# zenoran/sesameai-tts

Hardware: AMD Instinct MI355X
Metric: audio frames/sec (higher is better)
Workload: dtype bf16

## Files before the change

sesameai-tts_amd/csrc/dec_persist.cuh:

```cuda
#pragma once
#include "gemv.cuh"
#include "sampler.cuh"

#define DP_NB 256
#ifndef DP_NREP
#define DP_NREP 8
#endif
#define DP_TIMEOUT 5000000ull
#define DP_NL 4
#define DP_D 1024
#define DP_FFN 8192
#define DP_HD 128
#define DP_NQKV 1536
#define DP_WSM_ROWS 2560
#define DP_W2S_U4 (256L * 4 * 1024)
#define DP_W13P_U4 (256L * 4 * 32 * 64)
#define DP_LSLOTS 1088

typedef __attribute__((address_space(3))) uint32_t dp_lu32;
typedef __attribute__((address_space(3))) volatile uint32_t dp_lvu32;
typedef __attribute__((address_space(3))) u32x4_t dp_lu4;
typedef __attribute__((address_space(3))) unsigned short dp_lu16;
typedef __attribute__((address_space(3))) float dp_lf32;
typedef __attribute__((address_space(4))) const uint32_t dp_cu32;
// ... 14 lines not shown
    const bf16_t* proj_emb;
    const bf16_t* qkv0_tab;
    const bf16_t *hdec, *qd;
    const bf16_t *kc, *vc;
    long kv_layer_stride;
    float temperature; int topk;
    const bf16_t* noise;
    const uint64_t* rng;
    const SlotSampling* slot_tab;
    int slot_row0;
    const int* forced;
    int V, ncb;
    int* frame;
    bf16_t* logits_out;
    int cb_first, cb_last;
    dp_u64 *gQ, *gH1, *gH2, *gL, *gP;
    uint32_t* err;
    uint32_t* epoch;
    float eps;
    int trickle_sleep, poll_sleep;
    int fault;
    dp_u64* stamps;
};

#ifdef DP_TIMELINE
#define DP_STAMPS(a_) ((a_).stamps)
#define DP_FAULT(a_) ((a_).fault)
#else
#define DP_STAMPS(a_) ((dp_u64*)nullptr)
#define DP_FAULT(a_) 0
#endif
#define DP_OFF_K 0
#define DP_OFF_V 65536
#define DP_OFF_U 131072
#define DP_OFF_XA (DP_OFF_U)
#define DP_OFF_XC (DP_OFF_U + 2048)
#define DP_OFF_QB (DP_OFF_U + 4096)
#define DP_OFF_ATT (DP_OFF_U + 6144)
#define DP_CAND_SLOTS 2112
#define DP_OFF_CANDT (DP_OFF_U)
#define DP_OFF_CANDI (DP_OFF_U + DP_CAND_SLOTS * 4)
#define DP_OFF_LOGITS (DP_OFF_U + 16896)
#define DP_OFF_SMAX (DP_OFF_LOGITS + 5120)
#define DP_OFF_PS (DP_OFF_SMAX + 1024)
#define DP_OFF_MISC (DP_OFF_PS + 1024)
#define DP_LDS_BYTES (DP_OFF_MISC + 512)
static_assert(DP_OFF_CANDI + DP_CAND_SLOTS * 4 <= DP_OFF_LOGITS, "sampler candidate lists overrun the LDS logits");
#define DP_M_HL 0
#define DP_M_H0 16
#define DP_M_H1 18
#define DP_M_FXA 20
#define DP_M_FQ 21
#define DP_M_FXC 22
#define DP_M_FLG 23
#define DP_M_FTOK 24
#define DP_M_ATTN 25
#define DP_M_CD 26
#define DP_M_BAR 27
#define DP_M_ABORT 28
#define DP_M_TOK 29
#define DP_M_SBV 32
#define DP_M_SBI 36
#define DP_M_SN 40
#define DP_M_STOK 41
#define DP_M_SWTOT 42
#define DP_M_RNG 112
#define DP_M_SARG 116
#define DP_M_TILE 48

enum { DP_E_Q = 0, DP_E_H1 = 1, DP_E_P = 2, DP_E_H2 = 3, DP_E_L = 4 };
__device__ __forceinline__ uint32_t dp_tag(uint32_t base, int s, int l, int e) { return base + 1u + (uint32_t)((s * DP_NL + l) * 5 + e); }

__device__ __forceinline__ void dp_gran_store(dp_u64* p, uint32_t tag, uint32_t val) {
    __hip_atomic_store(p, ((dp_u64)tag << 32) | val, __ATOMIC_RELAXED, __HIP_MEMORY_SCOPE_AGENT);
}
__device__ __forceinline__ dp_u64 dp_gran_load(const dp_u64* p) { return __hip_atomic_load(p, __ATOMIC_RELAXED, __HIP_MEMORY_SCOPE_AGENT); }

__device__ __forceinline__ bool dp_give_up(dp_u64 t0, dp_lvu32* ab, uint32_t* err, uint32_t code, int lane) {
    if (*ab) return true;
    if (__builtin_amdgcn_s_memrealtime() - t0 > DP_TIMEOUT) {
        *ab = 1;
        if (lane == 0) atomicCAS(err, 0u, code);
        return true;
    }
    return false;
}

template <int N, bool AT_LEAST, class Issue>
__device__ __forceinline__ bool dp_wait(dp_lvu32* f, uint32_t tag, dp_lvu32* ab, uint32_t* err, uint32_t code, int lane, int sleep_units, Issue issue) {
    auto hit = [&]() { const uint32_t v = *f; return AT_LEAST ? (int32_t)(v - tag) >= 0 : v == tag; };
    int seen = (int)hit();
#pragma unroll
    for (int k = 0; k < N; ++k) {
        issue(k);
        const int nap = seen ? 0 : sleep_units;
        for (int z = 0; z < nap; ++z) __builtin_amdgcn_s_sleep(1);
        seen |= (int)hit();
    }
    seen = __builtin_amdgcn_readfirstlane(seen);
    if (!seen) {
        const dp_u64 t0 = __builtin_amdgcn_s_memrealtime();
        for (uint32_t spins = 1; !hit(); ++spins)
            if ((spins & 255u) == 0 && dp_give_up(t0, ab, err, code, lane)) return false;
    }
    asm volatile("" ::: "memory");
    return true;
}

template <int NL>
__device__ __forceinline__ bool dp_sweep(const dp_u64* g, int n_valid, uint32_t tag, uint32_t (&v)[2 * NL], int lane, dp_lvu32* ab, uint32_t* err,
                                         uint32_t code, int poll_sleep, dp_u64* passes = nullptr) {
    const dp_u64 t0 = __builtin_amdgcn_s_memrealtime();
    const int last_pair = (n_valid - 1) >> 1;
    for (;;) {
        if (passes && lane == 0) *passes += 1;
        u32x4_t x[NL];
#pragma unroll
        for (int j = 0; j < NL; ++j) {
            const dp_u64* p = g + 2 * min(j * 64 + lane, last_pair);
            asm volatile("global_load_dwordx4 %0, %1, off sc1" : "=v"(x[j]) : "v"(p) : "memory");
// ... 100 lines not shown
    mx0 = wave_max(mx0);
    float l0 = 0.f;
#pragma unroll
    for (int i = 0; i < NG; ++i) {
        s0[i] = (s0[i] == -INFINITY) ? 0.f : __expf(s0[i] - mx0);
        l0 += s0[i];
        if (sub == 0) myps[4 * i + grp] = s0[i];
    }
    l0 = wave_sum(l0) * (1.0f / 16.0f);
    asm volatile("s_waitcnt lgkmcnt(0)" ::: "memory");
    float o00 = 0.f, o01 = 0.f;
#pragma unroll
    for (int t4 = 0; t4 < NG; ++t4) {
        const u32x4_t p4 = *reinterpret_cast<const __attribute__((address_space(3))) u32x4_t*>(myps + 4 * t4);
        const float pw[4] = {__uint_as_float(p4.x), __uint_as_float(p4.y), __uint_as_float(p4.z), __uint_as_float(p4.w)};
        uint32_t vr[4];
#pragma unroll
        for (int u = 0; u < 4; ++u) vr[u] = vt[(4 * t4 + u) * 64 + lane];
#pragma unroll
        for (int u = 0; u < 4; ++u) { o00 += pw[u] * lo2f(vr[u]); o01 += pw[u] * hi2f(vr[u]); }
    }
    const float i0 = 1.0f / l0;
    att[h * 64 + lane] = pack_bf(o00 * i0, o01 * i0);
}
__device__ __forceinline__ void dp_attention_wave(char* lds, int wave, int l, int cb, int lane) {
    dp_lu32* misc = (dp_lu32*)(lds + DP_OFF_MISC);
    const int kvh = wave >> 2;
    const dp_lu4* qb = (const dp_lu4*)(lds + DP_OFF_QB);
    const dp_lu4* kt = (const dp_lu4*)(lds + DP_OFF_K + ((l * 2 + kvh) * 32) * 256);
    const dp_lu32* vt = (const dp_lu32*)(lds + DP_OFF_V + ((l * 2 + kvh) * 32) * 256);
    dp_lf32* ps = (dp_lf32*)(lds + DP_OFF_PS) + wave * 32;
    dp_lu32* att = (dp_lu32*)(lds + DP_OFF_ATT);
    dp_attention_head(qb, kt, vt, ps, att, wave, cb + 1, 0.08838834764831845f, lane);
    asm volatile("s_waitcnt lgkmcnt(0)" ::: "memory");
    if (lane == 0) __hip_atomic_fetch_add(misc + DP_M_ATTN, 1u, __ATOMIC_RELAXED, __HIP_MEMORY_SCOPE_WORKGROUP);
}

struct DpQuadSync {
    dp_lvu32* ctr; dp_lvu32* ab; uint32_t* err; int lane; uint32_t* phase; dp_u64* stamp;
    __device__ __forceinline__ void mark(int i) const { if (stamp != nullptr && lane == 0) stamp[i] = __builtin_amdgcn_s_memrealtime(); }
    __device__ __forceinline__ void operator()() const {
        asm volatile("s_waitcnt lgkmcnt(0)" ::: "memory");
        const uint32_t want = 4u * (++*phase);
        if (lane == 0) __hip_atomic_fetch_add((dp_lu32*)ctr, 1u, __ATOMIC_RELAXED, __HIP_MEMORY_SCOPE_WORKGROUP);
        const dp_u64 t0 = __builtin_amdgcn_s_memrealtime();
        for (uint32_t spins = 1; (int32_t)(*ctr - want) < 0; ++spins) {
            __builtin_amdgcn_s_sleep(2);
            if ((spins & 255u) == 0 && dp_give_up(t0, ab, err, 0xB00u, lane)) break;
        }
        asm volatile("" ::: "memory");
    }
};

template <bool DEBUG_OUT>
__device__ __forceinline__ int dp_sample_step(const DecPersistArgs& a, char* lds, int qw, int lane, int cu, int cb, int s, uint32_t* quad_phase) {
    dp_lu32* misc = (dp_lu32*)(lds + DP_OFF_MISC);
    dp_lvu32* ab = (dp_lvu32*)(misc + DP_M_ABORT);
    const int tid = qw * 64 + lane;
    if (DP_STAMPS(a) != nullptr && cu == 100 && tid == 0) DP_STAMPS(a)[s * 32 + 22] = __builtin_amdgcn_s_memrealtime();
    const dp_lu4* lg = (const dp_lu4*)(lds + DP_OFF_LOGITS);
    uint32_t w[2][4];
    {
        const uint4 v0 = dp_ldq(lg + tid);
        w[0][0] = v0.x; w[0][1] = v0.y; w[0][2] = v0.z; w[0][3] = v0.w;
        const uint4 v1 = tid < 64 ? dp_ldq(lg + 256 + tid) : make_uint4(0, 0, 0, 0);
        w[1][0] = v1.x; w[1][1] = v1.y; w[1][2] = v1.z; w[1][3] = v1.w;
    }
    if (DEBUG_OUT && a.logits_out != nullptr && cu == 0) {
        for (int i = lane; i < a.V; i += 64) a.logits_out[(long)cb * a.V + i] = ((const dp_lu16*)lg)[i];
    }
    SampleScratch sc;
    sc.cand_t = (lds_f32_t*)(lds + DP_OFF_CANDT); sc.cand_i = (lds_i32_t*)(lds + DP_OFF_CANDI); sc.s_max = (lds_u32_t*)(lds + DP_OFF_SMAX); sc.cand_q = (lds_f32_t*)(lds + DP_OFF_SMAX);
    sc.s_bv = (lds_f32_t*)(misc + DP_M_SBV); sc.s_bi = (lds_i32_t*)(misc + DP_M_SBI); sc.s_n = (lds_i32_t*)(misc + DP_M_SN);
    sc.s_tok = (lds_i32_t*)(misc + DP_M_STOK); sc.s_wtot = (lds_i32_t*)(misc + DP_M_SWTOT);
    DpQuadSync sync{(dp_lvu32*)(misc + DP_M_BAR), ab, a.err, lane, quad_phase, DP_STAMPS(a) != nullptr && cu == 100 && qw == 0 ? DP_STAMPS(a) + 4352 + s * 16 : nullptr};
    const uint64_t seed = (uint64_t)misc[DP_M_RNG] | ((uint64_t)misc[DP_M_RNG + 1] << 32), step = (uint64_t)misc[DP_M_RNG + 2] | ((uint64_t)misc[DP_M_RNG + 3] << 32);
    const int sV = (int)misc[DP_M_SARG], sK = (int)misc[DP_M_SARG + 2];
    const float sT = __uint_as_float(misc[DP_M_SARG + 1]);
    const bool sN = misc[DP_M_SARG + 3] != 0u;
    int tok = 0;
#ifdef DP_TIMELINE
    const int reps = (a.trickle_sleep & 128) ? 2 : 1;
#else
    constexpr int reps = 1;
#endif
#pragma unroll 1
    for (int r = 0; r < reps; ++r) {
        sync.mark(6);
        tok = sample_body<2>(w, sV, sT, sK, sN ? a.noise + (long)cb * sV : nullptr, seed, step, 0, cb, sc, tid, sync);
        sync.mark(7);
    }
    if (DP_STAMPS(a) != nullptr && cu == 100 && tid == 0) DP_STAMPS(a)[s * 32 + 23] = __builtin_amdgcn_s_memrealtime();
    if (tid == 0 && cu == 0) a.frame[cb] = tok;
    return tok;
}

typedef __attribute__((ext_vector_type(8))) __bf16 dp_bf16x8;
typedef __attribute__((ext_vector_type(4))) float dp_f32x4;
template <bool HAS_TILE, int NBK, int TROLE>
__device__ __forceinline__ void dp_compute_wave(const DecPersistArgs& a, char* lds, const int wave, const unsigned lane, const int cu, const uint32_t base,
                                                const uint32_t ropev) {
    constexpr bool HAS_B = !HAS_TILE;
    const bool is_x = HAS_TILE && TROLE == 1, is_a = HAS_TILE ? TROLE == 2 : TROLE == 1, is_b = HAS_B && !is_a;
    constexpr int NT = HAS_TILE ? 32 : 0, NCD = NT + NBK * 4, N1 = NCD / 3;
    dp_lu32* misc = (dp_lu32*)(lds + DP_OFF_MISC);
    dp_lvu32* ab = (dp_lvu32*)(misc + DP_M_ABORT);
    const int ts = a.trickle_sleep & 63;
    const int unit = is_a ? cu * 3 + (wave - 2) : cu * 2 + (wave - 5);
    auto my_block = [&](int b) { return wave < 4 ? wave + 4 * b : min((wave + 4) + 3 * b, wave == 6 ? 13 : 15); };
    const int hunit = is_x ? -1 : (wave < 6 ? cu * 4 + (wave - 2) : (cu < 2 ? 1024 + cu : -1));
    const int hrow0 = hunit < 0 ? 0 : 2 * hunit, hrow1 = hunit < 0 ? 0 : min(2 * hunit + 1, a.V - 1);
    uint4 wsa[2][2], wsb[HAS_B ? 2 : 1][2];
    uint4 wt[HAS_TILE ? 32 : 1];
    uint4 wd[NBK][4];

    auto ws_row = [&](int slot, int cb, int k) -> const bf16_t* {
        if (slot < DP_NL && !is_x) {
            if (is_a) {
                const int row = 2 * unit + (k >> 1);
                return a.wsm + ((long)slot * DP_WSM_ROWS + row) * DP_D;
            }
            return a.wsm + ((long)slot * DP_WSM_ROWS + DP_NQKV + 2 * unit + (k >> 1)) * DP_D;
        }
        return a.head_t + ((long)(cb - 1) * a.V + ((k >> 1) ? hrow1 : hrow0)) * DP_D;
    };
    auto load_wsa = [&](int slot, int cb, int k) { wsa[k >> 1][k & 1] = reinterpret_cast<const uint4*>(ws_row(slot, cb, k))[(k & 1) * 64 + lane]; };
    auto load_wsb = [&](int slot, int cb, int k) { wsb[HAS_B ? k >> 1 : 0][k & 1] = reinterpret_cast<const uint4*>(ws_row(slot, cb, k))[(k & 1) * 64 + lane]; };
// ... 97 lines not shown
                        tile[(lane >> 4) * 4 + 0] = acc[0]; tile[(lane >> 4) * 4 + 1] = acc[1];
                        tile[(lane >> 4) * 4 + 2] = acc[2]; tile[(lane >> 4) * 4 + 3] = acc[3];
                    }
                    asm volatile("s_waitcnt lgkmcnt(0)" ::: "memory");
                    if (lane < 8) {
                        const uint32_t hv = dp_swiglu(tile[lane], tile[8 + lane]);
                        ((dp_lu16*)(misc + DP_M_HL))[wave * 8 + lane] = (unsigned short)hv;
                    }
                }
                asm volatile("s_waitcnt lgkmcnt(0)" ::: "memory");
                if (lane == 0) __hip_atomic_fetch_add(misc + DP_M_CD, 1u, __ATOMIC_RELAXED, __HIP_MEMORY_SCOPE_WORKGROUP);
                {
                    const uint32_t want = 7u * (uint32_t)(it + 1);
                    const dp_u64 t0 = __builtin_amdgcn_s_memrealtime();
                    for (uint32_t spins = 1; (int32_t)(*(dp_lvu32*)(misc + DP_M_CD) - want) < 0; ++spins)
                        if ((spins & 255u) == 0 && dp_give_up(t0, ab, a.err, 0x950u, lane)) return;
                    asm volatile("" ::: "memory");
                }
                if (st0) DP_STAMPS(a)[4096 + s * 8 + 4] = __builtin_amdgcn_s_memrealtime();
                uint4 h[4];
#pragma unroll
                for (int q = 0; q < 4; ++q) h[q] = dp_ldq((const dp_lu4*)(misc + DP_M_HL) + q);
#pragma unroll
                for (int b = 0; b < NBK; ++b) {
                    const int n = my_block(b) * 64 + lane;
                    const float p = dp_down_partial(wd[b], h);
                    dp_gran_store(a.gP + ((long)(n >> 2) * 256 + cu) * 4 + (n & 3), dp_tag(base, s, l, DP_E_P), __float_as_uint(p));
                }
                if (st0) DP_STAMPS(a)[4096 + s * 8 + 5] = __builtin_amdgcn_s_memrealtime();
            }
        }
        {
            if (!dp_wait<1, false>((dp_lvu32*)(misc + DP_M_FXA), dp_tag(base, s, DP_NL - 1, DP_E_H2), ab, a.err, 0x960u, lane, ts, [&](int) {})) return;
            const bool st2 = DP_STAMPS(a) != nullptr && cu == 100 && lane == 0 && wave == 2;
            if (st2) DP_STAMPS(a)[s * 32 + 20] = __builtin_amdgcn_s_memrealtime();
            if (hunit >= 0) {
                const dp_lu4* xs = (const dp_lu4*)(lds + DP_OFF_XA);
                const uint4 x0 = dp_ldq(xs + lane), x1 = dp_ldq(xs + 64 + lane);
                uint4 r00 = wsa[0][0], r01 = wsa[0][1], r10 = wsa[1][0], r11 = wsa[1][1];
                if (HAS_B && is_b) { r00 = wsb[0][0]; r01 = wsb[0][1]; r10 = wsb[HAS_B ? 1 : 0][0]; r11 = wsb[HAS_B ? 1 : 0][1]; }
                float a0 = dot8(r00, x0, 0.f); a0 = dot8(r01, x1, a0);
                float a1 = dot8(r10, x0, 0.f); a1 = dot8(r11, x1, a1);
                a0 = wave_sum(a0); a1 = wave_sum(a1);
                if (lane < DP_NREP) dp_gran_store(a.gL + lane * DP_LSLOTS + hunit, dp_tag(base, s, DP_NL - 1, DP_E_L), pack_bf(a0, a1));
            }
            if (st2) DP_STAMPS(a)[s * 32 + 21] = __builtin_amdgcn_s_memrealtime();
            if (DP_STAMPS(a) != nullptr && s == 5 && lane == 0 && hunit >= 0) DP_STAMPS(a)[1024 + cu * 8 + wave] = __builtin_amdgcn_s_memrealtime();
            if (HAS_B) {
#pragma unroll
                for (int k = 0; k < 4; ++k) load_wsb(0, cb, k);
            }
        }
        if (!HAS_TILE) {
            if (!dp_wait<1, false>((dp_lvu32*)(misc + DP_M_FLG), dp_tag(base, s, DP_NL - 1, DP_E_L), ab, a.err, 0x970u, lane, ts, [&](int) {})) return;
            (void)dp_sample_step<false>(a, lds, wave - 4, (int)lane, cu, cb, s, &quad_phase);
            if (*ab) return;
        }
    }
}

#ifndef CSM_DEC_PERSIST_ELSEWHERE
static __global__ __launch_bounds__(512) void k_dec_persist(const DecPersistArgs a) {
    extern __shared__ __attribute__((aligned(16))) char lds[];
    const int wave = __builtin_amdgcn_readfirstlane(threadIdx.x >> 6), cu = blockIdx.x;
    const unsigned lane = threadIdx.x & 63;
    dp_lu32* misc = (dp_lu32*)(lds + DP_OFF_MISC);
    dp_lvu32* ab = (dp_lvu32*)(misc + DP_M_ABORT);
    uint32_t ropev = 0;
    if (wave >= 2 && wave <= 4 && lane < 32) {
        const int row = 2 * (cu * 3 + (wave - 2));
        const int e = (row < 1024 ? row : row - 1024) % DP_HD;
        ropev = reinterpret_cast<const uint32_t*>(a.rope)[lane * (DP_HD / 2) + e / 2];
    }
    for (int i = threadIdx.x; i < 128; i += 512) misc[i] = 0;
    for (int i = threadIdx.x; i < 2560 / 2; i += 512) ((dp_lu32*)(lds + DP_OFF_LOGITS))[i] = 0;
    for (int i = threadIdx.x; i < 131072 / 16; i += 512) dp_stq((dp_lu4*)lds + i, make_uint4(0, 0, 0, 0));
    __syncthreads();
    {
        const int npos = a.cb_first + 1;
        for (int i = threadIdx.x; i < DP_NL * 2 * npos * 16; i += 512) {
            const int c = i & 15, pos = (i >> 4) % npos, lk = (i >> 4) / npos;
            const long src = (long)(lk >> 1) * a.kv_layer_stride + ((long)(lk & 1) * 32 + pos) * DP_HD;
            dp_stq((dp_lu4*)(lds + DP_OFF_K + (lk * 32 + pos) * 256) + c, reinterpret_cast<const uint4*>(a.kc + src)[c]);
            dp_stq((dp_lu4*)(lds + DP_OFF_V + (lk * 32 + pos) * 256) + c, reinterpret_cast<const uint4*>(a.vc + src)[c]);
        }
        for (int i = threadIdx.x; i < 128; i += 512) dp_stq((dp_lu4*)(lds + DP_OFF_QB) + i, reinterpret_cast<const uint4*>(a.qd)[i]);
        if (threadIdx.x < 2) misc[DP_M_H0 + threadIdx.x] = reinterpret_cast<const uint32_t*>(a.hdec)[2 * cu + threadIdx.x];
        const uint32_t* se = a.slot_tab != nullptr ? reinterpret_cast<const uint32_t*>(a.slot_tab + a.slot_row0) : nullptr;
        const bool has = se != nullptr && se[1] != 0u, own = has && se[2] != 0u;
        if (threadIdx.x >= 64 && threadIdx.x < 68) misc[DP_M_RNG + threadIdx.x - 64] = own ? se[4 + threadIdx.x - 64] : (a.rng ? reinterpret_cast<const uint32_t*>(a.rng)[threadIdx.x - 64] : 0u);
        if (threadIdx.x == 128) { misc[DP_M_SARG] = (uint32_t)a.V; misc[DP_M_SARG + 1] = has ? se[0] : __float_as_uint(a.temperature); misc[DP_M_SARG + 2] = has ? se[1] : (uint32_t)a.topk; misc[DP_M_SARG + 3] = a.noise != nullptr; }
    }
    __syncthreads();
    const uint32_t base = dp_sload32(a.epoch);
    if (wave == 7) {
        __builtin_amdgcn_s_setprio(2);
        const int rep = cu % DP_NREP, ln = (int)lane;
        const dp_u64 *rgQ = a.gQ + rep * 768, *rgH1 = a.gH1 + rep * 512, *rgH2 = a.gH2 + rep * 512, *rgL = a.gL + rep * DP_LSLOTS;
        const dp_u64* rgP = a.gP + (long)cu * 1024;
        const int n_steps = a.cb_last - a.cb_first + 1;
        uint32_t quad_phase = 0;
        dp_flag((dp_lvu32*)(misc + DP_M_FQ), dp_tag(base, 0, 0, DP_E_Q));
        const bool st = DP_STAMPS(a) != nullptr && cu == 100 && lane == 0;
#define DP_STAMP(s_, i_) do { if (st) DP_STAMPS(a)[(s_) * 32 + (i_)] = __builtin_amdgcn_s_memrealtime(); } while (0)
        for (int s = 0; s < n_steps; ++s) {
            const int cb = a.cb_first + s;
            for (int l = 0; l < DP_NL; ++l) {
                if (l > 0) {
                    {
                        uint32_t v[8];
                        const uint4 g0 = reinterpret_cast<const uint4*>(a.norms + (long)(2 * l) * DP_D)[ln], g1 = reinterpret_cast<const uint4*>(a.norms + (long)(2 * l) * DP_D)[64 + ln];
                        if (!dp_sweep<4>(rgH2, 512, dp_tag(base, s, l - 1, DP_E_H2), v, ln, ab, a.err, 0x100u + l, a.poll_sleep)) return;
#pragma unroll
                        for (int j = 0; j < 4; ++j) { ((dp_lu32*)(lds + DP_OFF_XA))[2 * (j * 64 + ln)] = v[2 * j]; ((dp_lu32*)(lds + DP_OFF_XA))[2 * (j * 64 + ln) + 1] = v[2 * j + 1]; }
                        dp_norm_in_lds((dp_lu4*)(lds + DP_OFF_XA), g0, g1, a.eps, ln);
                        dp_flag((dp_lvu32*)(misc + DP_M_FXA), dp_tag(base, s, l - 1, DP_E_H2));
                        DP_STAMP(s, l * 4 + 0);
                    }
                    {
                        uint32_t v[12];
                        if (!dp_sweep<6>(rgQ, 768, dp_tag(base, s, l, DP_E_Q), v, ln, ab, a.err, 0x200u + l, a.poll_sleep, st ? DP_STAMPS(a) + s * 32 + 26 : nullptr)) return;
#pragma unroll
                        for (int j = 0; j < 4; ++j) { ((dp_lu32*)(lds + DP_OFF_QB))[2 * (j * 64 + ln)] = v[2 * j]; ((dp_lu32*)(lds + DP_OFF_QB))[2 * (j * 64 + ln) + 1] = v[2 * j + 1]; }
                        {
                            const int kvh = ln >> 5, wd_ = 2 * (ln & 31);
                            dp_lu32* kr = (dp_lu32*)(lds + DP_OFF_K + ((l * 2 + kvh) * 32 + cb) * 256);
                            dp_lu32* vr = (dp_lu32*)(lds + DP_OFF_V + ((l * 2 + kvh) * 32 + cb) * 256);
                            kr[wd_] = v[8]; kr[wd_ + 1] = v[9]; vr[wd_] = v[10]; vr[wd_ + 1] = v[11];
                        }
                        dp_flag((dp_lvu32*)(misc + DP_M_FQ), dp_tag(base, s, l, DP_E_Q));
                        DP_STAMP(s, l * 4 + 1);
                    }
                }
                dp_attention_wave(lds, 7, l, cb, ln);
                {
                    uint32_t v[8];
                    const uint4 g0 = reinterpret_cast<const uint4*>(a.norms + (long)(2 * l + 1) * DP_D)[ln], g1 = reinterpret_cast<const uint4*>(a.norms + (long)(2 * l + 1) * DP_D)[64 + ln];
                    if (!dp_sweep<4>(rgH1, 512, dp_tag(base, s, l, DP_E_H1), v, ln, ab, a.err, 0x300u + l, a.poll_sleep)) return;
#pragma unroll
                    for (int j = 0; j < 4; ++j) { ((dp_lu32*)(lds + DP_OFF_XC))[2 * (j * 64 + ln)] = v[2 * j]; ((dp_lu32*)(lds + DP_OFF_XC))[2 * (j * 64 + ln) + 1] = v[2 * j + 1]; }
                    dp_norm_in_lds((dp_lu4*)(lds + DP_OFF_XC), g0, g1, a.eps, ln);
                    dp_flag((dp_lvu32*)(misc + DP_M_FXC), dp_tag(base, s, l, DP_E_H1));
                    DP_STAMP(s, l * 4 + 2);
                }
                {
                    uint32_t v[16];
                    if (!dp_sweep<8>(rgP, 1024, dp_tag(base, s, l, DP_E_P), v, ln, ab, a.err, 0x400u + l, a.poll_sleep, st ? DP_STAMPS(a) + s * 32 + 27 : nullptr)) return;
                    float t0_, t1_;
                    dp_reduce_partials(v, t0_, t1_);
                    const uint32_t h1w = *(dp_lvu32*)(misc + DP_M_H1 + (ln & 1));
                    float y0, y1;
                    {
#pragma clang fp contract(off)
                        y0 = round_bf(t0_) + lo2f(h1w); y1 = round_bf(t1_) + hi2f(h1w);
                    }
                    const uint32_t pair = pack_bf(y0, y1);
                    if (ln < 2) misc[DP_M_H0 + ln] = pair;
                    if (ln < 2 * DP_NREP) dp_gran_store(a.gH2 + (ln >> 1) * 512 + 2 * cu + (ln & 1), dp_tag(base, s, l, DP_E_H2), pair);
                    DP_STAMP(s, l * 4 + 3);
                }
            }
            {
                uint32_t v[8];
                const uint4 g0 = reinterpret_cast<const uint4*>(a.dec_norm)[ln], g1 = reinterpret_cast<const uint4*>(a.dec_norm)[64 + ln];
                if (!dp_sweep<4>(rgH2, 512, dp_tag(base, s, DP_NL - 1, DP_E_H2), v, ln, ab, a.err, 0x500u, a.poll_sleep, st ? DP_STAMPS(a) + s * 32 + 25 : nullptr)) return;
#pragma unroll
                for (int j = 0; j < 4; ++j) { ((dp_lu32*)(lds + DP_OFF_XA))[2 * (j * 64 + ln)] = v[2 * j]; ((dp_lu32*)(lds + DP_OFF_XA))[2 * (j * 64 + ln) + 1] = v[2 * j + 1]; }
                dp_norm_in_lds((dp_lu4*)(lds + DP_OFF_XA), g0, g1, a.eps, ln);
                dp_flag((dp_lvu32*)(misc + DP_M_FXA), dp_tag(base, s, DP_NL - 1, DP_E_H2));
                DP_STAMP(s, 16);
                if (DP_STAMPS(a) != nullptr && s == 5 && lane == 0) DP_STAMPS(a)[1024 + 2048 + 256 + cu] = __builtin_amdgcn_s_memrealtime();
            }
            {
                uint32_t v[18];
                const int ng = (a.V + 1) / 2;
                if (!dp_sweep<9>(rgL, ng, dp_tag(base, s, DP_NL - 1, DP_E_L), v, ln, ab, a.err, 0x600u, a.poll_sleep, st ? DP_STAMPS(a) + s * 32 + 24 : nullptr)) return;
#pragma unroll
                for (int j = 0; j < 9; ++j) {
                    const int g0 = 2 * (j * 64 + ln);
                    if (g0 < ng) ((dp_lu32*)(lds + DP_OFF_LOGITS))[g0] = v[2 * j];
                    if (g0 + 1 < ng) ((dp_lu32*)(lds + DP_OFF_LOGITS))[g0 + 1] = v[2 * j + 1];
                }
                if ((a.V & 1) && ln == 0) ((dp_lu16*)(lds + DP_OFF_LOGITS))[a.V] = 0;
                dp_flag((dp_lvu32*)(misc + DP_M_FLG), dp_tag(base, s, DP_NL - 1, DP_E_L));
                DP_STAMP(s, 17);
                if (DP_STAMPS(a) != nullptr && s == 5 && lane == 0) DP_STAMPS(a)[1024 + 2048 + cu] = __builtin_amdgcn_s_memrealtime();
            }
            {
                const int tok = dp_sample_step<true>(a, lds, 3, ln, cu, cb, s, &quad_phase);
                if (*ab) return;
                DP_STAMP(s, 18);
                if (cb + 1 < a.ncb) {
                    int fed = a.forced ? a.forced[cb] : tok;
                    fed = min(max(fed, 0), a.V - 1);
                    const uint32_t* hrow = reinterpret_cast<const uint32_t*>(a.proj_emb + ((long)cb * a.V + fed) * DP_D);
                    const uint32_t* qrow = reinterpret_cast<const uint32_t*>(a.qkv0_tab + ((long)(cb - 1) * a.V + fed) * DP_NQKV);
                    uint32_t qv[12];
#pragma unroll
                    for (int j = 0; j < 12; ++j) qv[j] = qrow[j * 64 + ln];
                    const uint32_t hv = ln < 2 ? hrow[2 * cu + ln] : 0u;
#pragma unroll
                    for (int j = 0; j < 8; ++j) ((dp_lu32*)(lds + DP_OFF_QB))[j * 64 + ln] = qv[j];
#pragma unroll
                    for (int j = 8; j < 12; ++j)
                        ((dp_lu32*)(lds + (j < 10 ? DP_OFF_K : DP_OFF_V) + ((j & 1) * 32 + cb + 1) * 256))[ln] = qv[j];
                    if (ln < 2) misc[DP_M_H0 + ln] = hv;
                    dp_flag((dp_lvu32*)(misc + DP_M_FQ), dp_tag(base, s + 1, 0, DP_E_Q));
                    DP_STAMP(s, 19);
                }
            }
        }
        if (cu == 0 && lane == 0) __hip_atomic_store(a.epoch, base + (uint32_t)(n_steps * DP_NL * 5 + 8), __ATOMIC_RELAXED, __HIP_MEMORY_SCOPE_AGENT);
        return;
    }
    if (wave < 2) dp_compute_wave<true, 2, 1>(a, lds, wave, lane, cu, base, ropev);
    else if (wave < 4) dp_compute_wave<true, 2, 2>(a, lds, wave, lane, cu, base, ropev);
    else if (wave == 4) dp_compute_wave<false, 3, 1>(a, lds, wave, lane, cu, base, ropev);
    else dp_compute_wave<false, 3, 2>(a, lds, wave, lane, cu, base, ropev);
}
#endif

static __global__ void k_dp_pack_gateup(const bf16_t* w1, const bf16_t* w3, uint4* out) {
    const long i = (long)blockIdx.x * blockDim.x + threadIdx.x;
    if (i >= 256L * 4 * 32 * 64) return;
    const int lane = (int)(i & 63), t = (int)((i >> 6) & 31), q = (int)((i >> 11) & 3), c = (int)(i >> 13);
    const int r = lane & 15, pair = c * 32 + 8 * q + (r & 7);
    const bf16_t* w = r < 8 ? w1 : w3;
    out[i] = *reinterpret_cast<const uint4*>(w + (long)pair * DP_D + 32 * t + 8 * (lane >> 4));
}

static __global__ void k_dp_retile_w2(const bf16_t* w2, uint4* w2s) {
    const long i = (long)blockIdx.x * blockDim.x + threadIdx.x;
    if (i >= 256L * 4 * 1024) return;
    const int n = (int)(i % 1024), q = (int)((i / 1024) % 4), c = (int)(i / 4096);
    w2s[i] = *reinterpret_cast<const uint4*>(w2 + (long)n * DP_FFN + c * 32 + q * 8);
}

hipError_t csm_launch_dec_persist(const DecPersistArgs& p, hipStream_t st);
const void* csm_dec_persist_kernel();
```

sesameai-tts_amd/csrc/sampler.cuh:

```cuda
#pragma once
#include "common.cuh"
#include <math.h>

static __global__ __launch_bounds__(256) void k_embed_sum(const int* tokens , const uint8_t* mask ,
                                                   const bf16_t* text_emb, const bf16_t* audio_emb,
                                                   int audio_vocab, int text_vocab, int ncb, int d,
                                                   bf16_t* h ) {
    __shared__ const bf16_t* rows[64];
    const int m = blockIdx.x;
    if (threadIdx.x <= ncb && threadIdx.x < 64) {
        const int s = threadIdx.x;
        int t = tokens[(long)m * (ncb + 1) + s];
        const bf16_t* row = nullptr;
        if (mask[(long)m * (ncb + 1) + s]) {
            if (s < ncb) { t = min(max(t, 0), audio_vocab - 1); row = audio_emb + ((long)s * audio_vocab + t) * d; }
            else         { t = min(max(t, 0), text_vocab - 1);  row = text_emb + (long)t * d; }
        }
        rows[s] = row;
    }
    __syncthreads();
    for (int c = threadIdx.x; c < d / 8; c += 256) {
        float acc[8];
#pragma unroll
        for (int i = 0; i < 8; ++i) acc[i] = 0.f;
// ... 228 lines not shown
                    if (order_key(v) >= kth) sum += expf(v - mx);
                }
                sum = wave_sum(sum);
                const float logsum = round_bf(logf(round_bf(sum)));
                const float mx2 = round_bf(0.f - logsum);
                float s2 = 0.f;
                for (int c = lane; c < n; c += 64) {
                    const float v = sc.cand_t[c];
                    if (order_key(v) >= kth) s2 += expf(round_bf((v - mx) - logsum) - mx2);
                }
                s2 = wave_sum(s2);
                sync();
                for (int c = lane; c < n; c += 64) {
                    const float v = sc.cand_t[c];
                    if (order_key(v) < kth) continue;
                    const int idx = sc.cand_i[c];
                    const float p = round_bf(expf(round_bf((v - mx) - logsum) - mx2) / s2);
                    if (!(p > 0.f)) continue;
                    const float q = c < 256 ? sc.cand_q[c] : exp1_draw(idx, noise_row, seed, step, b, codebook);
                    const float r = round_bf(p / q);
                    if (r > best || (r == best && idx < best_idx)) { best = r; best_idx = idx; }
                }
            }
            sync.mark(5);
            const float wb = wave_max(best);
            best_idx = wave_min_i(best == wb ? best_idx : 0x7fffffff);
            if (lane == 0) *sc.s_tok = best_idx == 0x7fffffff ? 0 : best_idx;
        } else {
            for (int c = (wave - 1) * 64 + lane; c < min(n, 256); c += 192)
                sc.cand_q[c] = exp1_draw(sc.cand_i[c], noise_row, seed, step, b, codebook);
            sync();
        }
        sync();
        return *sc.s_tok;
    }
    {
        const float wb = wave_max(best);
        best_idx = wave_min_i(best == wb ? best_idx : 0x7fffffff);
        best = wb;
    }
    if (lane == 0) { sc.s_bv[wave] = best; sc.s_bi[wave] = best_idx; }
    sync();
    if (tid == 0) {
        float bv = sc.s_bv[0]; int bi = sc.s_bi[0];
        for (int x = 1; x < 4; ++x)
            if (sc.s_bv[x] > bv || (sc.s_bv[x] == bv && sc.s_bi[x] < bi)) { bv = sc.s_bv[x]; bi = sc.s_bi[x]; }
        if (bi == 0x7fffffff) bi = 0;
        *sc.s_tok = bi;
    }
    sync();
    return *sc.s_tok;
}

struct SyncThreads {
    __device__ __forceinline__ void operator()() const { __syncthreads(); }
    __device__ __forceinline__ void mark(int) const {}
};

template <int ITERS>
__global__ __launch_bounds__(256) void k_sample(const SampleArgs a) {
    __shared__ float cand_t[SAMPLE_MAX_ITERS * 512];
    __shared__ int cand_i[SAMPLE_MAX_ITERS * 512];
    __shared__ __attribute__((aligned(16))) uint32_t s_max[256];
    __shared__ float s_bv[4];
    __shared__ int s_bi[4];
    __shared__ int s_n, s_tok, s_wtot[4];
    const int b = blockIdx.x, tid = threadIdx.x, wave = tid >> 6, lane = tid & 63;
    const bf16_t* lg = a.logits + (long)b * a.ldl;
    uint64_t seed = a.rng ? a.rng[0] : 0, step = a.rng ? a.rng[1] : 0;
    float temperature = a.temperature;
    int topk = a.topk, seq = b;
    if (a.slot_tab != nullptr) {
        const SlotSampling e = a.slot_tab[a.slot_row0 + b];
        if (e.topk != 0) {
            temperature = e.temperature; topk = e.topk;
            if (e.own_rng) { seed = e.seed; step = e.counter; seq = 0; }
        }
    }
    uint32_t w[ITERS][4];
#pragma unroll
    for (int i = 0; i < ITERS; ++i) {
        const bool in = (i * 2048 + tid * 8) < a.ldl;
        const uint4 v = in ? reinterpret_cast<const uint4*>(lg + i * 2048)[tid] : make_uint4(0, 0, 0, 0);
        w[i][0] = v.x; w[i][1] = v.y; w[i][2] = v.z; w[i][3] = v.w;
    }
    SampleScratch sc;
    sc.cand_t = (lds_f32_t*)cand_t; sc.cand_i = (lds_i32_t*)cand_i; sc.s_max = (lds_u32_t*)s_max; sc.cand_q = (lds_f32_t*)s_max; sc.s_bv = (lds_f32_t*)s_bv;
    sc.s_bi = (lds_i32_t*)s_bi; sc.s_n = (lds_i32_t*)&s_n; sc.s_tok = (lds_i32_t*)&s_tok; sc.s_wtot = (lds_i32_t*)s_wtot;
    const int tok = sample_body<ITERS>(w, a.V, temperature, topk, a.noise ? a.noise + (long)b * a.V : nullptr, seed, step, seq,
                                       a.codebook, sc, tid, SyncThreads());
    if (tid == 0) a.frame[(long)b * a.ncb + a.codebook] = tok;
    if (a.emb_out) {
        int fed = a.forced ? a.forced[(long)b * a.ncb + a.codebook] : tok;
        fed = min(max(fed, 0), a.audio_vocab - 1);
        const uint4* src = reinterpret_cast<const uint4*>(a.audio_emb + ((long)a.codebook * a.audio_vocab + fed) * a.d);
        uint4* dst = reinterpret_cast<uint4*>(a.emb_out + (long)b * a.emb_stride);
        for (int c = tid; c < a.d / 8; c += 256) dst[c] = src[c];
        if (a.xn_out && wave == 0)
            rmsnorm_row_wave(reinterpret_cast<const bf16_t*>(src), a.d, a.xn_scale, a.xn_eps, a.xn_out + (long)b * a.xn_stride, lane);
        if (a.qkv0) {
            const int ld = a.nq + 2 * a.nkv, per_head = a.hd / 8;
            const uint4* row = reinterpret_cast<const uint4*>(a.qkv0 + (long)fed * ld);
            for (int c = tid; c < ld / 8; c += 256) {
                const uint4 v = row[c];
                if (c < a.nq / 8) reinterpret_cast<uint4*>(a.q_out + (long)b * a.nq)[c] = v;
                else {
// ... 71 lines not shown
```

Measured before the change: 370.0.

## Add single-wave top-k sampling fast path with helper waves computing draws

Replaces the four-wave quad-synchronised sampler in the persistent decoder with a single-wave front-end. It works directly on the register-resident logits and uses packed int16 ordering to find the k-th largest value, then compacts candidates with ballots. Helper waves are signalled through a new LDS go/arrive handshake to compute exponential draws in parallel. The usual case is meant to skip the LDS logits staging and the quad barriers; large top-k, NaN/inf, or too many candidates fall back to the old path. This adds protocol complexity and a bf16 semantics-matching risk.

Result: faster. 376.0 (median of 6 runs) (+1.6%).

```diff
diff --git a/sesameai-tts_amd/csrc/dec_persist.cuh b/sesameai-tts_amd/csrc/dec_persist.cuh
--- a/sesameai-tts_amd/csrc/dec_persist.cuh
+++ b/sesameai-tts_amd/csrc/dec_persist.cuh
@@ -90,13 +90,14 @@
 #define DP_M_FXA 20
 #define DP_M_FQ 21
 #define DP_M_FXC 22
-#define DP_M_FLG 23
 #define DP_M_FTOK 24
 #define DP_M_ATTN 25
 #define DP_M_CD 26
 #define DP_M_BAR 27
 #define DP_M_ABORT 28
 #define DP_M_TOK 29
+#define DP_M_SGO 30
+#define DP_M_SARR 31
 #define DP_M_SBV 32
 #define DP_M_SBI 36
 #define DP_M_SN 40
@@ -104,6 +105,7 @@
 #define DP_M_SWTOT 42
 #define DP_M_RNG 112
 #define DP_M_SARG 116
+#define DP_M_SDBG 120
 #define DP_M_TILE 48
 
 enum { DP_E_Q = 0, DP_E_H1 = 1, DP_E_P = 2, DP_E_H2 = 3, DP_E_L = 4 };
@@ -310,7 +312,32 @@
     }
 };
 
-template <bool DEBUG_OUT>
+__device__ __forceinline__ SampleScratch dp_sample_scratch(char* lds) {
+    dp_lu32* misc = (dp_lu32*)(lds + DP_OFF_MISC);
+    SampleScratch sc;
+    sc.cand_t = (lds_f32_t*)(lds + DP_OFF_CANDT); sc.cand_i = (lds_i32_t*)(lds + DP_OFF_CANDI); sc.s_max = (lds_u32_t*)(lds + DP_OFF_SMAX); sc.cand_q = (lds_f32_t*)(lds + DP_OFF_SMAX);
+    sc.s_bv = (lds_f32_t*)(misc + DP_M_SBV); sc.s_bi = (lds_i32_t*)(misc + DP_M_SBI); sc.s_n = (lds_i32_t*)(misc + DP_M_SN);
+    sc.s_tok = (lds_i32_t*)(misc + DP_M_STOK); sc.s_wtot = (lds_i32_t*)(misc + DP_M_SWTOT);
+    return sc;
+}
+
+enum { DP_SGO_LIST = 1, DP_SGO_FAST = 2, DP_SGO_QUAD = 3 };
+struct DpFrontHand {
+    dp_lvu32* go; dp_lvu32* arr; dp_lvu32* ab; uint32_t* err; int lane; uint32_t w0; uint32_t* arr_want; dp_u64* stamp;
+    __device__ __forceinline__ void mark(int i) const { if (stamp != nullptr && lane == 0) stamp[i] = __builtin_amdgcn_s_memrealtime(); }
+    __device__ __forceinline__ void publish_list() const { *arr_want += 3u; dp_flag(go, w0 + DP_SGO_LIST); }
+    __device__ __forceinline__ void publish_fast() const { dp_flag(go, w0 + DP_SGO_FAST); }
+    __device__ __forceinline__ bool wait_draws() const {
+        asm volatile("s_waitcnt lgkmcnt(0)" ::: "memory");
+        const uint32_t want = *arr_want;
+        const dp_u64 t0 = __builtin_amdgcn_s_memrealtime();
+        for (uint32_t spins = 1; (int32_t)(*arr - want) < 0; ++spins)
+            if ((spins & 255u) == 0 && dp_give_up(t0, ab, err, 0xB10u, lane)) return false;
+        asm volatile("" ::: "memory");
+        return true;
+    }
+};
+
 __device__ __forceinline__ int dp_sample_step(const DecPersistArgs& a, char* lds, int qw, int lane, int cu, int cb, int s, uint32_t* quad_phase) {
     dp_lu32* misc = (dp_lu32*)(lds + DP_OFF_MISC);
     dp_lvu32* ab = (dp_lvu32*)(misc + DP_M_ABORT);
@@ -324,13 +351,7 @@
         const uint4 v1 = tid < 64 ? dp_ldq(lg + 256 + tid) : make_uint4(0, 0, 0, 0);
         w[1][0] = v1.x; w[1][1] = v1.y; w[1][2] = v1.z; w[1][3] = v1.w;
     }
-    if (DEBUG_OUT && a.logits_out != nullptr && cu == 0) {
-        for (int i = lane; i < a.V; i += 64) a.logits_out[(long)cb * a.V + i] = ((const dp_lu16*)lg)[i];
-    }
-    SampleScratch sc;
-    sc.cand_t = (lds_f32_t*)(lds + DP_OFF_CANDT); sc.cand_i = (lds_i32_t*)(lds + DP_OFF_CANDI); sc.s_max = (lds_u32_t*)(lds + DP_OFF_SMAX); sc.cand_q = (lds_f32_t*)(lds + DP_OFF_SMAX);
-    sc.s_bv = (lds_f32_t*)(misc + DP_M_SBV); sc.s_bi = (lds_i32_t*)(misc + DP_M_SBI); sc.s_n = (lds_i32_t*)(misc + DP_M_SN);
-    sc.s_tok = (lds_i32_t*)(misc + DP_M_STOK); sc.s_wtot = (lds_i32_t*)(misc + DP_M_SWTOT);
+    const SampleScratch sc = dp_sample_scratch(lds);
     DpQuadSync sync{(dp_lvu32*)(misc + DP_M_BAR), ab, a.err, lane, quad_phase, DP_STAMPS(a) != nullptr && cu == 100 && qw == 0 ? DP_STAMPS(a) + 4352 + s * 16 : nullptr};
     const uint64_t seed = (uint64_t)misc[DP_M_RNG] | ((uint64_t)misc[DP_M_RNG + 1] << 32), step = (uint64_t)misc[DP_M_RNG + 2] | ((uint64_t)misc[DP_M_RNG + 3] << 32);
     const int sV = (int)misc[DP_M_SARG], sK = (int)misc[DP_M_SARG + 2];
@@ -534,9 +555,26 @@
             }
         }
         if (!HAS_TILE) {
-            if (!dp_wait<1, false>((dp_lvu32*)(misc + DP_M_FLG), dp_tag(base, s, DP_NL - 1, DP_E_L), ab, a.err, 0x970u, lane, ts, [&](int) {})) return;
-            (void)dp_sample_step<false>(a, lds, wave - 4, (int)lane, cu, cb, s, &quad_phase);
-            if (*ab) return;
+            dp_lvu32* go = (dp_lvu32*)(misc + DP_M_SGO);
+            const uint32_t w0 = 4u * (uint32_t)(s + 1);
+            if (!dp_wait<1, true>(go, w0 + DP_SGO_LIST, ab, a.err, 0x970u, lane, ts, [&](int) {})) return;
+            const bool st4 = DP_STAMPS(a) != nullptr && cu == 100 && lane == 0 && wave == 4;
+            if (st4) DP_STAMPS(a)[s * 32 + 28] = __builtin_amdgcn_s_memrealtime();
+            uint32_t state = *go - w0;
+            if (state != DP_SGO_QUAD) {
+                const bool sN = misc[DP_M_SARG + 3] != 0u;
+                const uint64_t seed = (uint64_t)misc[DP_M_RNG] | ((uint64_t)misc[DP_M_RNG + 1] << 32), step = (uint64_t)misc[DP_M_RNG + 2] | ((uint64_t)misc[DP_M_RNG + 3] << 32);
+                sample_wave_draws(dp_sample_scratch(lds), wave - 4, 3, (int)lane, sN ? a.noise + (long)cb * (int)misc[DP_M_SARG] : nullptr, seed, step, 0, cb);
+                asm volatile("s_waitcnt lgkmcnt(0)" ::: "memory");
+                if (lane == 0) __hip_atomic_fetch_add(misc + DP_M_SARR, 1u, __ATOMIC_RELAXED, __HIP_MEMORY_SCOPE_WORKGROUP);
+                if (st4) DP_STAMPS(a)[s * 32 + 29] = __builtin_amdgcn_s_memrealtime();
+                if (!dp_wait<1, true>(go, w0 + DP_SGO_FAST, ab, a.err, 0x980u, lane, ts, [&](int) {})) return;
+                state = *go - w0;
+            }
+            if (state == DP_SGO_QUAD) {
+                (void)dp_sample_step(a, lds, wave - 4, (int)lane, cu, cb, s, &quad_phase);
+                if (*ab) return;
+            }
         }
     }
 }
@@ -571,7 +609,7 @@
         const uint32_t* se = a.slot_tab != nullptr ? reinterpret_cast<const uint32_t*>(a.slot_tab + a.slot_row0) : nullptr;
         const bool has = se != nullptr && se[1] != 0u, own = has && se[2] != 0u;
         if (threadIdx.x >= 64 && threadIdx.x < 68) misc[DP_M_RNG + threadIdx.x - 64] = own ? se[4 + threadIdx.x - 64] : (a.rng ? reinterpret_cast<const uint32_t*>(a.rng)[threadIdx.x - 64] : 0u);
-        if (threadIdx.x == 128) { misc[DP_M_SARG] = (uint32_t)a.V; misc[DP_M_SARG + 1] = has ? se[0] : __float_as_uint(a.temperature); misc[DP_M_SARG + 2] = has ? se[1] : (uint32_t)a.topk; misc[DP_M_SARG + 3] = a.noise != nullptr; }
+        if (threadIdx.x == 128) { misc[DP_M_SARG] = (uint32_t)a.V; misc[DP_M_SARG + 1] = has ? se[0] : __float_as_uint(a.temperature); misc[DP_M_SARG + 2] = has ? se[1] : (uint32_t)a.topk; misc[DP_M_SARG + 3] = a.noise != nullptr; misc[DP_M_SDBG] = a.logits_out != nullptr; }
     }
     __syncthreads();
     const uint32_t base = dp_sload32(a.epoch);
@@ -581,7 +619,7 @@
         const dp_u64 *rgQ = a.gQ + rep * 768, *rgH1 = a.gH1 + rep * 512, *rgH2 = a.gH2 + rep * 512, *rgL = a.gL + rep * DP_LSLOTS;
         const dp_u64* rgP = a.gP + (long)cu * 1024;
         const int n_steps = a.cb_last - a.cb_first + 1;
-        uint32_t quad_phase = 0;
+        uint32_t quad_phase = 0, arr_want = 0;
         dp_flag((dp_lvu32*)(misc + DP_M_FQ), dp_tag(base, 0, 0, DP_E_Q));
         const bool st = DP_STAMPS(a) != nullptr && cu == 100 && lane == 0;
 #define DP_STAMP(s_, i_) do { if (st) DP_STAMPS(a)[(s_) * 32 + (i_)] = __builtin_amdgcn_s_memrealtime(); } while (0)
@@ -653,24 +691,52 @@
                 DP_STAMP(s, 16);
                 if (DP_STAMPS(a) != nullptr && s == 5 && lane == 0) DP_STAMPS(a)[1024 + 2048 + 256 + cu] = __builtin_amdgcn_s_memrealtime();
             }
+            int tok;
+            bool own_code;
             {
                 uint32_t v[18];
                 const int ng = (a.V + 1) / 2;
+                const int sV = (int)misc[DP_M_SARG], sK = (int)misc[DP_M_SARG + 2];
+                const float sT = __uint_as_float(misc[DP_M_SARG + 1]);
+                const bool dbg = misc[DP_M_SDBG] != 0u && cu == 0;
+                const bool quad0 = !(sK > 1 && min(sK, sV) <= 128);
                 if (!dp_sweep<9>(rgL, ng, dp_tag(base, s, DP_NL - 1, DP_E_L), v, ln, ab, a.err, 0x600u, a.poll_sleep, st ? DP_STAMPS(a) + s * 32 + 24 : nullptr)) return;
-#pragma unroll
-                for (int j = 0; j < 9; ++j) {
-                    const int g0 = 2 * (j * 64 + ln);
-                    if (g0 < ng) ((dp_lu32*)(lds + DP_OFF_LOGITS))[g0] = v[2 * j];
-                    if (g0 + 1 < ng) ((dp_lu32*)(lds + DP_OFF_LOGITS))[g0 + 1] = v[2 * j + 1];
-                }
-                if ((a.V & 1) && ln == 0) ((dp_lu16*)(lds + DP_OFF_LOGITS))[a.V] = 0;
-                dp_flag((dp_lvu32*)(misc + DP_M_FLG), dp_tag(base, s, DP_NL - 1, DP_E_L));
                 DP_STAMP(s, 17);
                 if (DP_STAMPS(a) != nullptr && s == 5 && lane == 0) DP_STAMPS(a)[1024 + 2048 + cu] = __builtin_amdgcn_s_memrealtime();
+                auto logits_to_lds = [&]() {
+#pragma unroll
+                    for (int j = 0; j < 9; ++j) {
+                        const int g0 = 2 * (j * 64 + ln);
+                        if (g0 < ng) ((dp_lu32*)(lds + DP_OFF_LOGITS))[g0] = v[2 * j];
+                        if (g0 + 1 < ng) ((dp_lu32*)(lds + DP_OFF_LOGITS))[g0 + 1] = v[2 * j + 1];
+                    }
+                    if ((sV & 1) && ln == 0) ((dp_lu16*)(lds + DP_OFF_LOGITS))[sV] = 0;
+                };
+                const uint32_t w0 = 4u * (uint32_t)(s + 1);
+                if (quad0 || dbg) logits_to_lds();
+                if (quad0) dp_flag((dp_lvu32*)(misc + DP_M_SGO), w0 + DP_SGO_QUAD);
+                if (dbg) {
+                    asm volatile("s_waitcnt lgkmcnt(0)" ::: "memory");
+                    for (int i = ln; i < sV; i += 64) a.logits_out[(long)cb * sV + i] = ((const dp_lu16*)(lds + DP_OFF_LOGITS))[i];
+                }
+                tok = SAMPLE_WAVE_FALLBACK;
+                if (!quad0) {
+                    const DpFrontHand hand{(dp_lvu32*)(misc + DP_M_SGO), (dp_lvu32*)(misc + DP_M_SARR), ab, a.err, ln, w0, &arr_want,
+                                           st ? DP_STAMPS(a) + 4352 + s * 16 + 8 : nullptr};
+                    tok = sample_wave_front<9>(v, sV, sT, min(sK, sV), dp_sample_scratch(lds), ln, hand);
+                    if (tok == SAMPLE_WAVE_ABORT) return;
+                    if (tok == SAMPLE_WAVE_FALLBACK) {
+                        if (!dbg) logits_to_lds();
+                        dp_flag((dp_lvu32*)(misc + DP_M_SGO), w0 + DP_SGO_QUAD);
+                    }
+                }
+                own_code = tok != SAMPLE_WAVE_FALLBACK;
+                if (!own_code) {
+                    tok = dp_sample_step(a, lds, 3, ln, cu, cb, s, &quad_phase);
+                    if (*ab) return;
+                }
             }
             {
-                const int tok = dp_sample_step<true>(a, lds, 3, ln, cu, cb, s, &quad_phase);
-                if (*ab) return;
                 DP_STAMP(s, 18);
                 if (cb + 1 < a.ncb) {
                     int fed = a.forced ? a.forced[cb] : tok;
@@ -690,6 +756,7 @@
                     dp_flag((dp_lvu32*)(misc + DP_M_FQ), dp_tag(base, s + 1, 0, DP_E_Q));
                     DP_STAMP(s, 19);
                 }
+                if (own_code && cu == 0 && ln == 0) a.frame[cb] = tok;
             }
         }
         if (cu == 0 && lane == 0) __hip_atomic_store(a.epoch, base + (uint32_t)(n_steps * DP_NL * 5 + 8), __ATOMIC_RELAXED, __HIP_MEMORY_SCOPE_AGENT);
diff --git a/sesameai-tts_amd/csrc/sampler.cuh b/sesameai-tts_amd/csrc/sampler.cuh
--- a/sesameai-tts_amd/csrc/sampler.cuh
+++ b/sesameai-tts_amd/csrc/sampler.cuh
@@ -304,6 +304,124 @@
     return *sc.s_tok;
 }
 
+#define SAMPLE_WAVE_FALLBACK (-1)
+#define SAMPLE_WAVE_ABORT (-2)
+#define SAMPLE_WAVE_DUMP 255
+typedef short s16x2_t __attribute__((ext_vector_type(2)));
+__device__ __forceinline__ s16x2_t pk_order(uint32_t w) {
+    const s16x2_t x = __builtin_bit_cast(s16x2_t, w);
+    const s16x2_t sg = x >> 15;
+    return (x ^ (sg & (short)0x7fff)) - sg;
+}
+template <int NL, class Hand>
+__device__ __forceinline__ int sample_wave_front(const uint32_t (&v)[2 * NL], int V, float temperature, int k, const SampleScratch& sc, int lane, Hand hand) {
+    s16x2_t o[2 * NL], z[2 * NL];
+#pragma unroll
+    for (int r = 0; r < 2 * NL; ++r) o[r] = z[r] = pk_order(v[r]);
+#pragma unroll
+    for (int j = 0; j < NL; ++j)
+        if (256 * (j + 1) > V) {
+#pragma unroll
+            for (int h = 0; h < 2; ++h) {
+                const int idx0 = 4 * (j * 64 + lane) + 2 * h;
+                const uint32_t bits = __builtin_bit_cast(uint32_t, o[2 * j + h]);
+                const uint32_t in = (idx0 < V ? bits & 0xffffu : 0u) | (idx0 + 1 < V ? bits & 0xffff0000u : 0u);
+                z[2 * j + h] = __builtin_bit_cast(s16x2_t, in);
+                o[2 * j + h] = __builtin_bit_cast(s16x2_t, in | (idx0 < V ? 0u : 0x8000u) | (idx0 + 1 < V ? 0u : 0x80000000u));
+            }
+        }
+    s16x2_t gmx = o[0], zmax = z[0], zmin = z[0];
+#pragma unroll
+    for (int r = 1; r < 2 * NL; ++r) {
+        gmx = __builtin_elementwise_max(gmx, o[r]);
+        zmax = __builtin_elementwise_max(zmax, z[r]);
+        zmin = __builtin_elementwise_min(zmin, z[r]);
+    }
+    if (__ballot(max(zmax.x, zmax.y) > 0x7f80 || min(zmin.x, zmin.y) < -0x7f80) != 0ull) return SAMPLE_WAVE_FALLBACK;
+    const uint32_t gm[2] = {(uint32_t)((int)gmx.x + 32768), (uint32_t)((int)gmx.y + 32768)};
+    const uint32_t L = kth_largest_key<2>(gm, k);
+    hand.mark(0);
+    const uint32_t margin = 2u * (uint32_t)ceilf(fmaxf(temperature, 1.0f)) + 2u;
+    const uint32_t Lm = L > margin ? L - margin : 1u;
+    const short lms = (short)((int)Lm - 32768);
+    const s16x2_t lm2 = {lms, lms};
+    const int idx_lane = 4 * lane;
+    int n = 0;
+#pragma unroll
+    for (int j = 0; j < NL; ++j) {
+        const uint32_t d0 = __builtin_bit_cast(uint32_t, __builtin_elementwise_sub_sat(o[2 * j], lm2));
+        const uint32_t d1 = __builtin_bit_cast(uint32_t, __builtin_elementwise_sub_sat(o[2 * j + 1], lm2));
+        const bool f[4] = {(int)(d0 << 16) >= 0, (int)d0 >= 0, (int)(d1 << 16) >= 0, (int)d1 >= 0};
+        uint32_t p = (uint32_t)n;
+#pragma unroll
+        for (int e = 0; e < 4; ++e) {
+            const unsigned long long m = __ballot(f[e]);
+            p = __builtin_amdgcn_mbcnt_hi((unsigned)(m >> 32), __builtin_amdgcn_mbcnt_lo((unsigned)m, p));
+            n += __popcll(m);
+        }
+#pragma unroll
+        for (int e = 0; e < 4; ++e) {
+            const uint32_t w = v[2 * j + (e >> 1)];
+            const uint32_t idx = (uint32_t)(idx_lane | (256 * j + e));
+            sc.cand_i[f[e] ? (int)p : SAMPLE_WAVE_DUMP] = (int)((e & 1) ? ((w & 0xffff0000u) | idx) : ((w << 16) | idx));
+            p += f[e] ? 1u : 0u;
+        }
+    }
+    if (n > 128) return SAMPLE_WAVE_FALLBACK;
+    if (lane == 0) *sc.s_n = n;
+    hand.publish_list();
+    hand.mark(1);
+    float tv[2]; int ix[2]; uint32_t ck[2];
+#pragma unroll
+    for (int u = 0; u < 2; ++u) {
+        const int c = u * 64 + lane;
+        const bool live = c < n;
+        const uint32_t w = (uint32_t)sc.cand_i[live ? c : 0];
+        tv[u] = round_bf(__uint_as_float(w & 0xffff0000u) / temperature);
+        ix[u] = (int)(w & 0xffffu) | (c << 16);
+        ck[u] = live ? order_key(tv[u]) : 0u;
+    }
+    const uint32_t kth = n > k ? kth_largest_key<2>(ck, k) : 0u;
+    const bool keep0 = ck[0] != 0u && ck[0] >= kth, keep1 = ck[1] != 0u && ck[1] >= kth;
+    const unsigned long long m0 = __ballot(keep0), m1 = __ballot(keep1);
+    const int kept0 = __popcll(m0), kept = kept0 + __popcll(m1);
+    hand.mark(2);
+    if (kept > 64) {
+        if (!hand.wait_draws()) return SAMPLE_WAVE_ABORT;
+        return SAMPLE_WAVE_FALLBACK;
+    }
+    hand.publish_fast();
+    const int p0 = (int)__builtin_amdgcn_mbcnt_hi((unsigned)(m0 >> 32), __builtin_amdgcn_mbcnt_lo((unsigned)m0, 0u));
+    const int p1 = kept0 + (int)__builtin_amdgcn_mbcnt_hi((unsigned)(m1 >> 32), __builtin_amdgcn_mbcnt_lo((unsigned)m1, 0u));
+    if (keep0) { sc.cand_t[128 + p0] = tv[0]; sc.cand_i[128 + p0] = ix[0]; }
+    if (keep1) { sc.cand_t[128 + p1] = tv[1]; sc.cand_i[128 + p1] = ix[1]; }
+    const bool live = lane < kept;
+    const float x = sc.cand_t[128 + (live ? lane : 0)];
+    const int pk = sc.cand_i[128 + (live ? lane : 0)];
+    const float mx = wave_max(live ? x : -INFINITY);
+    const float sum = wave_sum(live ? expf(x - mx) : 0.f);
+    const float logsum = round_bf(logf(round_bf(sum)));
+    const float mx2 = round_bf(0.f - logsum);
+    const float e3 = live ? expf(round_bf((x - mx) - logsum) - mx2) : 0.f;
+    const float s2 = wave_sum(e3);
+    hand.mark(3);
+    if (!hand.wait_draws()) return SAMPLE_WAVE_ABORT;
+    hand.mark(4);
+    int best_idx = 0x7fffffff;
+    float best = -INFINITY;
+    const float p = round_bf(e3 / s2);
+    if (live && p > 0.f) { best = round_bf(p / sc.cand_q[pk >> 16]); best_idx = pk & 0xffff; }
+    const float wb = wave_max(best);
+    best_idx = wave_min_i(best == wb ? best_idx : 0x7fffffff);
+    return best_idx == 0x7fffffff ? 0 : best_idx;
+}
+__device__ __forceinline__ void sample_wave_draws(const SampleScratch& sc, int hw, int nh, int lane, const bf16_t* noise_row, uint64_t seed, uint64_t step,
+                                                  int b, int codebook) {
+    const int n = min(*sc.s_n, 256);
+    for (int c = hw * 64 + lane; c < n; c += 64 * nh)
+        sc.cand_q[c] = exp1_draw(sc.cand_i[c] & 0xffff, noise_row, seed, step, b, codebook);
+}
+
 struct SyncThreads {
     __device__ __forceinline__ void operator()() const { __syncthreads(); }
     __device__ __forceinline__ void mark(int) const {}
```
